# andreicuceu/vega

Measured on AMD Instinct MI355X. Metric: model+chi2 evals/sec (Lya auto+cross), higher is better.
Workload: dtype f64

## Files before the change

vega_amd/csrc/vegamx.hip:

```cpp
#include "vmx_device.h"
#include "vmx_fit.h"
#include "vmx_ensemble.h"
#include "vmx_nested.h"
#include "vmx_smc.h"

#include <atomic>
#include <cmath>
#include <chrono>
#include <thread>
#include <algorithm>
#include <cstdio>
#include <cstdlib>
#include <cstring>
#include <map>
#include <mutex>
#include <queue>
#include <utility>
#include <string>
#include <vector>

#ifndef VMX_MAX_LANES
#define VMX_MAX_LANES 2
#endif

// ... 1566 lines not shown
    DevBuf<double> xtab_key;
    int n_xtab = 0;
    int const_hint = 0;
    int fv_n = 0;
    struct GkSpec { double rp, rt, mock_rp, mock_rt; };
    std::vector<GkSpec> gk_tables;
    std::vector<double> h_k, h_mu;

    int n_coef = 0, ncp = 0, n_knots = 0;
    DevBuf<double> op;
    bool op_set[VMX_MAX_ELL] = {false, false, false, false};
    bool extrapolate = false;
    double x0[VMX_MAX_ELL] = {0}, h[VMX_MAX_ELL] = {0};

    std::vector<PipeDev> pipes;
    std::vector<double> h_r, h_mu_c, h_z, h_relz, h_lnrelz, h_lnrelz2, h_growth;
    DevBuf<double> cr, cmu, crp, crt, cz, crelz, clnrelz, clnrelz2, cgrowth;
    DevBuf<PipeDev> d_pipes;
    std::vector<PkGroup> pk_groups;
    DevBuf<PkGroup> d_pk_groups;
    std::vector<int32_t> pk_members, pk_poly, pk_static;
    DevBuf<int32_t> d_pk_members, d_pk_poly, d_pk_static, d_pipe_active;
    DevBuf<double> poly_coef, poly_bins;
    int64_t poly_bins_total = 0;
    int n_active = 0;
    bool poly_dirty = true;

    std::vector<ItemHost*> items;
    std::vector<MetalHost*> metals;
    DevBuf<ItemDev> d_items;
    DevBuf<MetalDev> d_metals;
    std::vector<double> h_bb, h_odd, h_odd_op;
    std::map<int, int64_t> odd_op_off;
    DevBuf<double> bb_basis, odd_coef, odd_op, odd_dyn, sn_a;
    int sn_n = 0; double sn_tau0 = 0.0, sn_dtau = 1.0;

    std::vector<int32_t> prior_slot;
    std::vector<double> prior_mean, prior_sigma;
    DevBuf<int32_t> d_prior_slot;
    DevBuf<double> d_prior_mean, d_prior_sigma;

    DevBuf<double> gcinv, gres, gz;
    int g_n = 0, g_ld = 0;

    int n_params = 0, max_batch = 0, model_size = 0, slab_rows = 0;
    int pad_l = 0, pad_r = 0;
// ... 574 lines not shown
    for (size_t i = 0; i < e->gk_tables.size(); ++i) {
        const auto& g = e->gk_tables[i];
        if (g.rp == bin_size_rp && g.rt == bin_size_rt && g.mock_rp == mock_size_rp && g.mock_rt == mock_size_rt) return (int)i;
    }
    e->gk_tables.push_back({bin_size_rp, bin_size_rt, mock_size_rp, mock_size_rt});
    return (int)e->gk_tables.size() - 1;
}

int vmx_add_gk_table(vmx_engine* e, double bin_size_rp, double bin_size_rt)
{
    return vmx_add_gk_table_mock(e, bin_size_rp, bin_size_rt, 0.0, 0.0);
}

int vmx_add_pipeline(vmx_engine* e, const vmx_pipe_desc* desc, int32_t n, const double* r, const double* mu,
                     const double* z, const double* rel_z_evol, const double* xi_growth)
{
    if (!e || e->finalized || !desc || n <= 0) return fail(-1, "invalid argument: vmx_add_pipeline");
    if (desc->n_ell < 1 || desc->n_ell > VMX_MAX_ELL) return fail(-1, "invalid argument: n_ell");
    if (desc->gk_table >= (int)e->gk_tables.size()) return fail(-1, "invalid argument: gk_table id");
    if (desc->mock_los_slot >= 0 && !(desc->mock_los_size > 0.0)) return fail(-1, "invalid argument: mock_los_size");
    if (desc->n_smooth < 0 || desc->n_smooth > VMX_MAX_SMOOTH) return fail(-1, "invalid argument: n_smooth");
    PipeDev p{};
    p.d = *desc;
    p.poly_basis = -1; p.col = -1; p.poly_bins_off = -1; p.odd_dyn_off = -1;
    if (!p.d.same_tracer && ((!p.d.tracer[0].is_lya && p.d.tracer[1].is_lya) ||
                             (p.d.tracer[0].is_lya == p.d.tracer[1].is_lya && p.d.tracer[0].discrete &&
                              !p.d.tracer[1].discrete))) {
        std::swap(p.d.tracer[0], p.d.tracer[1]);
        p.tracers_swapped = 1;
    }
    p.n = n;
    p.coord_off = (int64_t)e->h_r.size();
    e->h_r.insert(e->h_r.end(), r, r + n);
    e->h_mu_c.insert(e->h_mu_c.end(), mu, mu + n);
    e->h_z.insert(e->h_z.end(), z, z + n);
    e->h_relz.insert(e->h_relz.end(), rel_z_evol, rel_z_evol + n);
    for (int i = 0; i < n; ++i) { e->h_lnrelz.push_back(std::log(rel_z_evol[i])); e->h_lnrelz2.push_back(std::log(rel_z_evol[i])); }
    p.rp_absmin = 1e300; p.rp_absmax = 0.0; p.rt_min = 1e300; p.rt_max = 0.0;
    for (int i = 0; i < n; ++i) {
        if (r[i] == 0.0) continue;
        const double rp = std::fabs(r[i] * mu[i]), rt = r[i] * std::sqrt(std::max(0.0, 1.0 - mu[i] * mu[i]));
        p.rp_absmin = std::min(p.rp_absmin, rp); p.rp_absmax = std::max(p.rp_absmax, rp);
        p.rt_min = std::min(p.rt_min, rt); p.rt_max = std::max(p.rt_max, rt);
    }
    if (p.rp_absmin > p.rp_absmax) { p.rp_absmin = 0.0; p.rt_min = 0.0; }
    e->h_growth.insert(e->h_growth.end(), xi_growth, xi_growth + n);
    e->pipes.push_back(p);
// ... 407 lines not shown
    REQUIRE(e && invcov && n > 0, "vmx_set_global_invcov");
    drop_lane(e);
    HIP_OK(hipSetDevice(e->device));
    const std::vector<double> half = half_form(invcov, n);
    if (e->finalized) {
        REQUIRE(e->g_n == n, "global inverse covariance size changed");
        HIP_OK(hipStreamSynchronize(e->stream));
        HIP_OK(hipMemcpy2D(e->gcinv.p, (size_t)e->g_ld * sizeof(double), half.data(), (size_t)n * sizeof(double),
                           (size_t)n * sizeof(double), n, hipMemcpyHostToDevice));
        return 0;
    }
    e->g_n = n; e->g_ld = vmx_pad(n);
    return upload_padded(e->gcinv, half.data(), n, n, e->g_ld);
}

int vmx_add_prior(vmx_engine* e, int32_t slot, double mean, double sigma)
{
    REQUIRE(e && !e->finalized && slot >= 0 && sigma != 0.0, "vmx_add_prior");
    e->prior_slot.push_back(slot); e->prior_mean.push_back(mean); e->prior_sigma.push_back(sigma);
    return 0;
}

static int poly_basis_build(vmx_engine* e);
static int xi_sum_plan(vmx_engine* e);

int vmx_finalize(vmx_engine* e, int32_t n_params, int32_t max_batch)
{
    REQUIRE(e && !e->finalized, "vmx_finalize");
    REQUIRE(n_params > 0 && max_batch > 0, "n_params / max_batch");
    REQUIRE(e->nk > 0 && !e->pipes.empty() && !e->items.empty(), "template, pipelines and items are required");
    REQUIRE(e->items.size() <= 16, "at most 16 correlation items");
    REQUIRE(e->pipes.size() * sizeof(PipeDev) <= 48 * 1024, "too many pipelines for the prologue's descriptor stage");
    for (int i = 0; i < VMX_MAX_ELL; ++i) REQUIRE(e->op_set[i], "all four FFTLog operators are required");
    HIP_OK(hipSetDevice(e->device));
    const int Bm = max_batch;
    e->n_params = n_params; e->max_batch = Bm;
    e->slab_rows = Bm > 1024 ? Bm : 1024;
    e->fact_slab_rows = std::max(1024, std::min(4 * Bm, 8192));
    if (getenv("VMX_NO_GRAPH")) e->use_graphs = false;
    if (getenv("VMX_TRACE_HOST")) e->trace_host = true;
    {
        int cus = 256;
        if (hipDeviceGetAttribute(&cus, hipDeviceAttributeMultiprocessorCount, e->device) != hipSuccess || cus <= 0) { (void)hipGetLastError(); cus = 256; }
        e->quad_blocks = 2 * cus;
    }
    if (getenv("VMX_NO_TAB2")) e->no_tab2 = true;
// ... 390 lines not shown
    if (getenv("VMX_NO_DONE_WORD") || hipHostGetDevicePointer((void**)&e->dpin_done, e->pin_done, 0) != hipSuccess) { (void)hipGetLastError(); e->dpin_done = nullptr; }
    if (!getenv("VMX_NO_ZERO_COPY") &&
        (hipHostGetDevicePointer((void**)&e->dpin_theta, e->pin_theta, 0) != hipSuccess ||
         hipHostGetDevicePointer((void**)&e->dpin_chi2, e->pin_chi2, 0) != hipSuccess ||
         hipHostGetDevicePointer((void**)&e->dpin_status, e->pin_status, 0) != hipSuccess)) {
        (void)hipGetLastError();
        e->dpin_theta = nullptr; e->dpin_chi2 = nullptr; e->dpin_status = nullptr;
    }

    e->quad_eligible = e->gcinv.p == nullptr && e->items.size() <= 16;
    for (auto* it : e->items) {
        int na = 0;
        if (it->dev.n_bb[VMX_BB_POST_MUL]) e->quad_eligible = false;
        for (int q = 0; q < it->dev.n_bb[VMX_BB_POST_ADD]; ++q) {
            if (it->dev.bb[VMX_BB_POST_ADD][q].func != VMX_BB_POLY) e->quad_eligible = false;
            na += it->dev.bb[VMX_BB_POST_ADD][q].n_coef;
        }
        if (na > VMX_MAX_QUAD_COEF) e->quad_eligible = false;
    }
    if (getenv("VMX_NO_QUAD")) e->quad_eligible = false;

    HIP_OK(hipStreamSynchronize(e->stream));
    e->finalized = true;
    if (poly_basis_build(e) || xi_sum_plan(e)) { e->finalized = false; return -2; }
    return 0;
}

int vmx_model_size(vmx_engine* e) { return e ? e->model_size : -1; }

int vmx_pipeline_column(vmx_engine* e, int32_t pipeline)
{
    REQUIRE(e && e->finalized && pipeline >= 0 && pipeline < (int)e->pipes.size(), "vmx_pipeline_column");
    return e->pipes[pipeline].col >= 0 ? e->pipes[pipeline].col : -3 - e->n_active;
}

constexpr double QUAD_ENTRY_STAGES = 4.0, QUAD_SKEW = 0.12;
constexpr bool QUAD_K_BANDS = true;

static vmx_engine::QuadList* quad_build_tape(vmx_engine* e, int B)
{
    const int tn = (B + GEMM_BN - 1) / GEMM_BN;
    std::vector<vmx_plan::TapeProblem> probs;
    for (auto* it : e->items) probs.push_back({it->dev.nq, it->dev.nq_pad});
    vmx_plan::Tape T = vmx_plan::plan_quad_tape(probs, tn, e->quad_blocks, QUAD_ENTRY_STAGES, QUAD_SKEW, GEMM_BM, GEMM_BK, QUAD_K_BANDS);
    auto* ql = new vmx_engine::QuadList();
    ql->n_blocks = T.n_blocks;
    ql->n_entries = (int)T.n_slots;
// ... 111 lines not shown
        DevBuf<int32_t> d_ok;
        if (d_ok.upload(ok.data(), ok.size())) return -2;
        int max_n = 0;
        for (int p : e->pk_static) max_n = std::max(max_n, (int)e->pipes[p].n);
        hipLaunchKernelGGL(k_poly_bins, dim3((max_n + 255) / 256, ns, 3), dim3(256), 0, e->stream, e->dev, e->d_pk_static.p,
                           e->poly_bins.p, d_ok.p);
        e->route_setup |= VMX_ROUTE_POLY_BINS;
        HIP_OK(hipGetLastError());
        HIP_OK(hipStreamSynchronize(e->stream));
        HIP_OK(hipMemcpy(ok.data(), d_ok.p, ok.size() * sizeof(int32_t), hipMemcpyDeviceToHost));
        bool changed = false;
        for (int sb = 0; sb < ns; ++sb)
            if (!ok[sb] && e->pipes[e->pk_static[sb]].poly_bins_off >= 0) { e->pipes[e->pk_static[sb]].poly_bins_off = -1; changed = true; }
        if (changed) HIP_OK(hipMemcpy(e->d_pipes.p, e->pipes.data(), e->pipes.size() * sizeof(PipeDev), hipMemcpyHostToDevice));
    }
    HIP_OK(hipStreamSynchronize(e->stream));
    for (int p : e->pk_static) (e->pipes[p].poly_bins_off >= 0 ? e->xi_static_bins : e->xi_static_taps).push_back(p);
    std::vector<int32_t> a = e->xi_static_taps, b = e->xi_static_bins;
    a.push_back(-1); b.push_back(-1);
    if (e->d_xi_static_taps.upload(a.data(), a.size()) || e->d_xi_static_bins.upload(b.data(), b.size())) return -2;
    return 0;
}

static void launch_metal_kron(vmx_engine* e, const EngineDev& D, ItemHost* it, int B)
{
    int item = 0;
    for (size_t q = 0; q < e->items.size(); ++q) if (e->items[q] == it) item = (int)q;
    size_t shmem = 0;
    for (auto* m : it->metals) {
        if (!m->dev.kron_a) continue;
        const int n = m->dev.kron_nrp * m->dev.kron_nrt;
        shmem = std::max(shmem, (size_t)(2 * n + std::max(m->dev.kron_nrp * m->dev.kron_nrp, m->dev.kron_nrt * m->dev.kron_nrt)) * sizeof(double));
    }
    if (shmem == 0) return;
    ScopedTimer t(e, KC_METAL);
    if (!e->kron_attr) { (void)hipFuncSetAttribute((const void*)k_metal_kron, hipFuncAttributeMaxDynamicSharedMemorySize, 160 * 1024); e->kron_attr = true; }
    hipLaunchKernelGGL(k_metal_kron, dim3(B, (unsigned)it->metals.size()), dim3(256), shmem, e->cur, D, item, B);
}

static bool xi_plain_args(vmx_engine* e, XiPlainArgs& A)
{
    if (e->items.size() > VMX_MAX_GROUP || e->extrapolate || e->direct) return false;
    for (size_t q = 0; q < e->items.size(); ++q) {
        const ItemHost* it = e->items[q];
        const ItemDev& d = it->dev;
        if (!it->lean_pair || d.add_vec || d.n_bb[VMX_BB_PRE_MUL] || d.n_bb[VMX_BB_PRE_ADD]) return false;
        const PipeDev& Ps = e->pipes[d.d.pipe_smooth];
        const PipeDev& Pp = e->pipes[d.d.pipe_peak];
        if (Ps.d.n_ell != Pp.d.n_ell || Ps.d.single_ell >= 0 || Pp.d.single_ell >= 0 || Ps.col < 0 || Pp.col < 0) return false;
        XiPlainItem& I = A.it[q];
        I.coord_off = Pp.coord_off; I.q_x0 = it->q_x0.p; I.q_x = it->q_x.p;
        I.n_model = d.d.n_model; I.nq = d.nq; I.nq_pad = d.nq_pad; I.pipe_s = d.d.pipe_smooth; I.pipe_p = d.d.pipe_peak;
        I.col_s = Ps.col; I.col_p = Pp.col; I.n_ell = Ps.d.n_ell; I.split_evol = Pp.split_evol; I.bao_slot = d.d.bao_amp_slot;
        I.item = (int32_t)q;
        I.radiation = Ps.d.radiation;
    }
    return true;
}

static int xi_sum_plan(vmx_engine* e)
{
    e->sums_dirty = false;
    e->lean_groups.clear(); e->static_groups.clear(); e->static_single.clear(); e->lean_single.clear();
    e->sums_any = false;
    const int np = (int)e->pipes.size();
    struct Role { int item = -1, fkind = 0, findex = 0, metal = -1, refs = 0; bool plain = true; };
    std::vector<Role> role(np);
    int metal_base = 0;
    for (int q = 0; q < (int)e->items.size(); ++q) {
        const ItemHost* it = e->items[q];
        const vmx_item_desc& d = it->dev.d;
        auto take = [&](int p, int fkind, int findex, int metal, bool plain) {
            if (p < 0 || p >= np) return;
            Role& r = role[p];
            r.refs += 1; r.item = q; r.fkind = fkind; r.findex = findex; r.metal = metal; r.plain = r.plain && plain;
        };
        take(d.pipe_smooth, 0, 0, -1, true);
        if (d.pipe_peak != d.pipe_smooth) take(d.pipe_peak, 1, d.bao_amp_slot, -1, true);
// ... 3101 lines not shown
    }
    else if (what == 6) { src = e->scal.p; count = (int64_t)B * (int64_t)e->pipes.size() * VMX_NS; }
    else if (what == 7) {
        static_assert(VMX_DEBUG_NS == VMX_NS, "vegamx.h states the row length of the scalars");
#define VMX_SCALAR_INDEX(name) S_##name,
        const int idx[] = {VMX_NS, VMX_DEBUG_SCALARS(VMX_SCALAR_INDEX)};
#undef VMX_SCALAR_INDEX
        const int64_t n = sizeof(idx) / sizeof(idx[0]);
        if (capacity < n) { fail(-1, "invalid argument: capacity too small"); return -1; }
        for (int64_t i = 0; i < n; ++i) out[i] = idx[i];
        return n;
    }
    else if (what == 8) {
        if (index < 0 || index >= (int)e->pipes.size()) { fail(-1, "invalid argument: pipeline index"); return -1; }
        const PipeDev& P = e->pipes[index];
        const double* arr[8] = {e->cr.p, e->crp.p, e->crt.p, e->cz.p, e->crelz.p, e->clnrelz.p, e->clnrelz2.p, e->cgrowth.p};
        if ((int64_t)8 * P.n > capacity) { fail(-1, "invalid argument: capacity too small"); return -1; }
        for (int a = 0; a < 8; ++a)
            if (hipMemcpy(out + (size_t)a * P.n, arr[a] + P.coord_off, (size_t)P.n * sizeof(double), hipMemcpyDeviceToHost) != hipSuccess) { fail(-2, "hipMemcpy"); return -2; }
        return (int64_t)8 * P.n;
    }
    else if (what == 9) {
        if (index < 0 || index >= (int)e->pipes.size()) { fail(-1, "invalid argument: pipeline index"); return -1; }
        if (capacity < 30) { fail(-1, "invalid argument: capacity too small"); return -1; }
        const EngineDev& D = e->dev;
        const PipeDev& P = e->pipes[index];
        int64_t n = 0;
        out[n++] = D.n_coef; out[n++] = D.ncp; out[n++] = D.same_grid; out[n++] = D.extrapolate; out[n++] = e->n_active;
        for (int l = 0; l < VMX_MAX_ELL; ++l) { out[n++] = D.x0[l]; out[n++] = D.h[l]; out[n++] = D.inv_h[l]; out[n++] = D.xlast[l]; }
        out[n++] = P.col; out[n++] = P.n; out[n++] = P.n_pad; out[n++] = P.split_evol; out[n++] = P.poly_basis;
        out[n++] = P.poly_bins_off >= 0 ? 1 : 0; out[n++] = P.odd_x0; out[n++] = P.odd_h; out[n++] = P.odd_ncoef;
        return n;
    }
    else if (what == 10 || what == 11) {
        if (index < 0 || index >= (int)e->items.size()) { fail(-1, "invalid argument: item index"); return -1; }
        const ItemHost* it = e->items[index];
        if (e->last_full || e->last_form == 0 || !it->q_x.p || !it->q_x0.p) { fail(-1, "the last evaluation was not a chi2-only evaluation of the quadratic form: no x' - x0'"); return -1; }
        src = what == 10 ? it->q_x.p : it->q_x0.p; count = (what == 10 ? (int64_t)B : 1) * it->dev.nq_pad;
    }
    else if (what == 12) {
        if (index < 0 || index >= (int)e->pipes.size()) { fail(-1, "invalid argument: pipeline index"); return -1; }
        const PipeDev& P = e->pipes[index];
        if (P.poly_bins_off < 0 || !e->poly_bins.p) { fail(-1, "none: the pipeline has no static basis on its bins"); return -1; }
        src = e->poly_bins.p + P.poly_bins_off; count = (int64_t)3 * P.n_pad;
    }
    else if (what == 13 || what == 14 || what == 18 || what == 19) {
        const bool lean = what < 18, describe = what == 13 || what == 18;
        const int ng = (int)(lean ? e->lean_groups.size() : e->static_groups.size());
        if (describe && (index < 0 || index >= ng)) {
            if (capacity < 1) { fail(-1, "invalid argument: capacity too small"); return -1; }
            out[0] = ng;
            return 1;
        }
        if (index < 0 || index >= ng) { fail(-1, "invalid argument: group index"); return -1; }
// ... 141 lines not shown
```

vega_amd/csrc/vmx_device.h:

```cpp
#pragma once
#include <hip/hip_runtime.h>
#include <stdint.h>
#include "../../include/vegamx.h"
#include "vmx_plan.h"

#define VMX_NS 40
#define VMX_PAD 32
#define VMX_MAX_BB 32
#define VMX_MAX_METALS 64
#define VMX_MAX_QUAD_COEF 64
#define VMX_MAX_GROUP 8
#define VMX_MAX_MARG 16

enum {
    S_BIAS1 = 0, S_BB1, S_BIAS2, S_BB2,
    S_UV_BG, S_UV_BP, S_UV_LAM, S_HE_BG, S_HE_LAM,
    S_HCD_B, S_HCD_BB, S_HCD_L0,
    S_GA, S_GB, S_EA, S_EB,
    S_AQ1, S_AQ2, S_AKV, S_AAV, S_ABV, S_AKP,
    S_VD1, S_VD2,
    S_AP, S_AT, S_DRP, S_EV1A, S_EV1B, S_EV2A, S_EV2B,
    S_RAD_S, S_RAD_A, S_RAD_L, S_RAD_D, S_RAD_IL, S_RAD_ID,
    S_NO_RULE
};

static inline int vmx_pad(int n) { return (n + VMX_PAD - 1) / VMX_PAD * VMX_PAD; }

struct PipeDev {
    vmx_pipe_desc d;
    int32_t n;
    int32_t n_pad;
    int64_t coord_off;
    int64_t xi_off;
    double rp_absmin, rp_absmax, rt_min, rt_max;
    int32_t col;
    int32_t poly_basis;
    int64_t poly_bins_off;
    int32_t split_evol;
    int32_t tracers_swapped;
    int32_t odd_rel, odd_asy, odd_ncoef;
    int32_t odd_slot[5];
    int64_t odd_off;
    int64_t odd_dyn_off;
    int32_t odd_dyn_ld;
    double odd_x0, odd_h;
};

struct BBTermDev {
    int32_t func, n_coef;
    int32_t slot[16];
    int64_t basis_off;
};

struct MetalDev {
    vmx_metal_desc d;
    int64_t mat_off;
    int32_t mat_ld;
    int64_t xim_off;
    const double* svec;
    const double* basis;
// ... 56 lines not shown
    const double* mu;
    const double* mu_img;
    vmx_plan::MuTierDesc mu_tier[vmx_plan::MU_TIERS];
    const double* mu_img_w;
    const double* sq1mmu2;
    const double* lnmu;
    const double* wl;
    const double* fv_x; const double* fv_f; int32_t fv_n;
    const double* gk;
    double* xtab;
    const int32_t* const_slots; int32_t n_const_slots;
    const int32_t* xtab_pipe; const int32_t* xtab_partner; int32_t n_xtab; int32_t xtab_level; double* xtab_key; double* xtab_k;
    int32_t xtab_block0;
    const double* gk_mom;
    int32_t n_gk;
    int32_t n_coef, ncp;
    int32_t extrapolate;
    double x0[VMX_MAX_ELL], h[VMX_MAX_ELL], xlast[VMX_MAX_ELL], inv_h[VMX_MAX_ELL];
    int same_grid;
    int32_t n_pipe;
    int32_t n_active;
    const double* poly_coef;
    const double* poly_bins;
    int32_t n_static;
    const PipeDev* pipes;
    const double* crp; const double* crt;
    const double* cr; const double* cmu; const double* cz; const double* crelz; const double* clnrelz; const double* cgrowth;
    const double* clnrelz2;
    int32_t n_items;
    const ItemDev* items;
    const MetalDev* metals;
    int32_t n_metals_total;
    const double* bb_basis;
    const double* odd_coef;
    const double* odd_dyn;
    const double* sn_a; int32_t sn_n; double sn_tau0, sn_dtau;
    int32_t n_priors;
    const int32_t* prior_slot; const double* prior_mean; const double* prior_sigma;
    int32_t n_params;
    const double* theta;
    const double* theta_host; double* theta_copy; double* chi2_host; int32_t* status_host;
    int32_t src_host;
    double* scal;
    double* metal_bias;
    double beta_override; int32_t beta_override_on;
    double* pl;
// ... 2702 lines not shown
                const double v = (part[tid][0] + part[tid][1]) + (part[tid][2] + part[tid][3]);
                pr = sx[r] * (2.0 * (v - g.lin[r]));
            }
            for (int off = 32; off > 0; off >>= 1) pr += __shfl_down(pr, off, 64);
            if (tid == 0) {
                *(volatile double*)&g.part[blockIdx.x] = pr;
                if (blockIdx.x == 0 && item) {
                    *(volatile int32_t*)D.status_host = D.status[0];
                    D.k_live[2] = D.coef_win[0]; D.k_live[3] = D.coef_win[1]; D.coef_win[0] = 0x7fffffff; D.coef_win[1] = -1;
                    xtab_key_store(D);
                }
            }
        }
        return;
    }
    if (tid < t) {
        const int r = blockIdx.x + tid * gridDim.x;
        const double v = (part[tid][0] + part[tid][1]) + (part[tid][2] + part[tid][3]);
        if constexpr (FUSED) post_bin(D, D.items[item], 0, r, v);
        else Dp[r] = v;
    }
}

__device__ inline double legendre_even(int e, double x)
{
    const double x2 = x * x;
    switch (e) {
        case 0: return 1.0;
        case 1: return 0.5 * (3.0 * x2 - 1.0);
        case 2: return 0.125 * ((35.0 * x2 - 30.0) * x2 + 3.0);
        default: return 0.0625 * (((231.0 * x2 - 315.0) * x2 + 105.0) * x2 - 5.0);
    }
}

template <bool STATIC_BASIS>
__device__ __forceinline__ double spline_legendre(const EngineDev& D, const PipeDev& P, int b, int nB, double x, double rmu,
                                                  double a0, double a1, double a2, bool& oob)
{
    const vmx_pipe_desc& d = P.d;
    const int n_ell = d.n_ell, single_ell = d.single_ell;
    const size_t ncols = (size_t)nB * D.n_active;
    const size_t col = (size_t)(P.col >= 0 ? P.col : 0) * nB + b;
    const double* cf[4];
    double tt[4];
    bool on[4];
#pragma unroll
    for (int e = 0; e < 4; ++e) {
        const int ee = e < n_ell ? e : 0;
        const bool inside = D.extrapolate || !(x < D.x0[ee] || x > D.xlast[ee]);
        on[e] = e < n_ell && inside;
        if (e < n_ell && !inside) oob = true;
        const double u = (x - D.x0[ee]) * D.inv_h[ee];
        int j = (int)floor(u);
        if (j < 0) j = 0;
        if (j > D.n_coef - 4) j = D.n_coef - 4;
        if (!(u == u)) j = 0;
        tt[e] = u - (double)j;
        cf[e] = STATIC_BASIS ? D.poly_coef + ((size_t)ee * D.n_static + P.poly_basis) * 3 * D.ncp + j
                             : D.coef + ((size_t)ee * ncols + col) * D.ncp + j;
    }
    double tap[4][4];
    if (STATIC_BASIS) {
#pragma unroll
        for (int e = 0; e < 4; ++e)
#pragma unroll
            for (int q = 0; q < 4; ++q)
                tap[e][q] = fma(a2, cf[e][2 * D.ncp + q], fma(a1, cf[e][D.ncp + q], a0 * cf[e][q]));
    } else {
#pragma unroll
        for (int e = 0; e < 4; ++e)
#pragma unroll
            for (int q = 0; q < 4; ++q) tap[e][q] = cf[e][q];
    }
    double xi = 0.0;
#pragma unroll
    for (int e = 0; e < 4; ++e) {
        const double t = tt[e], t2 = t * t, t3 = t2 * t;
        const double omt = 1.0 - t;
        const double w0 = omt * omt * omt;
        const double w1 = 3.0 * t3 - 6.0 * t2 + 4.0;
        const double w2 = -3.0 * t3 + 3.0 * t2 + 3.0 * t + 1.0;
        const double s = (tap[e][0] * w0 + tap[e][1] * w1 + tap[e][2] * w2 + tap[e][3] * t3) * (1.0 / 6.0);
        if (on[e]) {
            if (single_ell >= 0) { if (e == single_ell) xi = s; }
            else xi += s * legendre_even(e, rmu);
        }
    }
    return xi;
}

__device__ __forceinline__ void kaiser_coefficients(const vmx_pipe_desc& d, const double* sc, double& a0, double& a1, double& a2)
{
    double c01 = sc[S_BIAS1], c02 = sc[S_BIAS2];
    const double c11 = sc[S_BB1], c12 = d.same_tracer ? sc[S_BB1] : sc[S_BB2];
    if (d.same_tracer) c02 = c01;
    a0 = c01 * c02; a1 = fma(c01, c12, c11 * c02); a2 = c11 * c12;
}

template <int MODE>
__device__ __forceinline__ double xi_bin_value(const EngineDev& D, int p, int b, int bin, int nB, bool& oob_out)
{
    const PipeDev& P = D.pipes[p];
    const vmx_pipe_desc& d = P.d;
    const double* sc = D.scal + ((size_t)b * D.n_pipe + p) * VMX_NS;
    const size_t c = P.coord_off + bin;
    const double r = D.cr[c], rp0 = D.crp[c], rt0 = D.crt[c];
    const double lnrelz = D.clnrelz[c], growth = D.cgrowth[c];
    const double drp = sc[S_DRP], s_ap = sc[S_AP], s_at = sc[S_AT];
// ... 106 lines not shown
    bool oob;
    D.xi[P.xi_off + (size_t)b * P.n_pad + bin] = xi_bin_value<2>(D, p, b, bin, (int)gridDim.z, oob);
}

__global__ __launch_bounds__(256) void k_poly_bins(EngineDev D, const int32_t* pipes, double* out, int32_t* ok)
{
    const int sb = blockIdx.y, p = pipes[sb], i = blockIdx.z;
    const PipeDev& P = D.pipes[p];
    const int bin = blockIdx.x * 256 + threadIdx.x;
    if (bin >= P.n || P.poly_bins_off < 0) return;
    const size_t c = P.coord_off + bin;
    const double r = D.cr[c], rp0 = D.crp[c], rt0 = D.crt[c];
    double xi = 0.0;
    bool oob = false;
    if (r != 0.0) {
        const double rr2 = fma(rp0, rp0, rt0 * rt0);
        if (rr2 != 0.0)
            xi = spline_legendre<true>(D, P, 0, 1, 0.5 * log(rr2), rp0 * vmx_rsqrt(rr2), i == 0 ? 1.0 : 0.0, i == 1 ? 1.0 : 0.0,
                                       i == 2 ? 1.0 : 0.0, oob);
    }
    if (oob) ok[sb] = 0;
    out[P.poly_bins_off + (size_t)i * P.n_pad + bin] = xi;
}

__global__ __launch_bounds__(256) void k_xi_assemble_quad(EngineDev D, int item0, int store_xi)
{
    const ItemDev& it = D.items[item0 + blockIdx.z];
    const int b = blockIdx.y, nB = gridDim.y;
    const int i = blockIdx.x * 256 + threadIdx.x;
    if (i >= it.nq_pad) return;
    const double* t = D.theta + (size_t)b * D.n_params;
    double v = 0.0;
    if (i < it.d.n_model) {
        const PipeDev& Pp = D.pipes[it.d.pipe_peak];
        const PipeDev& Ps = D.pipes[it.d.pipe_smooth];
        bool oob_p, oob_s;
        double xs, xp;
        if (it.plain_pair) {
            const size_t c = Pp.coord_off + i;
            const double r = D.cr[c], rp0 = D.crp[c], rt0 = D.crt[c];
            const double* scp = D.scal + ((size_t)b * D.n_pipe + it.d.pipe_peak) * VMX_NS;
            const double* scs = D.scal + ((size_t)b * D.n_pipe + it.d.pipe_smooth) * VMX_NS;
            const double ev = (Pp.split_evol ? vmx_exp(fma(scp[S_EV1A], D.clnrelz[c], scp[S_EV2A] * D.clnrelz2[c]))
                                             : vmx_exp((scp[S_EV1A] + scp[S_EV2A]) * D.clnrelz[c])) * D.cgrowth[c];
            xs = 0.0; xp = 0.0; oob_p = false; oob_s = false;
            if (r != 0.0) {
#pragma unroll
                for (int half = 0; half < 2; ++half) {
                    const double* sc = half ? scp : scs;
                    const double rrp = sc[S_AP] * (rp0 + sc[S_DRP]), rrt = sc[S_AT] * rt0;
                    const double rr2 = fma(rrp, rrp, rrt * rrt);
                    if (rr2 != 0.0) {
                        const double v = spline_legendre<false>(D, half ? Pp : Ps, b, nB, 0.5 * vmx_log(rr2), rrp * vmx_rsqrt(rr2),
                                                                0.0, 0.0, 0.0, half ? oob_p : oob_s);
                        if (half) xp = v * ev; else xs = v * ev;
                    }
                }
            }
        } else {
            xs = xi_bin_value<0>(D, it.d.pipe_smooth, b, i, nB, oob_s);
            xp = xi_bin_value<0>(D, it.d.pipe_peak, b, i, nB, oob_p);
        }
        if (oob_p || oob_s) atomicOr(&D.status[b], VMX_STATUS_BOUNDS);
        if (store_xi) {
            D.xi[Ps.xi_off + (size_t)b * Ps.n_pad + i] = xs;
            D.xi[Pp.xi_off + (size_t)b * Pp.n_pad + i] = xp;
        }
        const double bao = t[it.d.bao_amp_slot];
        v = fma(bao, xp, xs);
        if (it.add_vec) v = fma(it.add_slot >= 0 ? t[it.add_slot] : it.add_default, it.add_vec[i], v);
        if (it.n_bb[VMX_BB_PRE_MUL]) v *= bb_total(D, it, VMX_BB_PRE_MUL, t, i, it.d.n_model);
        if (it.n_bb[VMX_BB_PRE_ADD]) v += (1.0 + bao) * bb_total(D, it, VMX_BB_PRE_ADD, t, i, it.d.n_model);
        v -= it.q_x0[i];
    } else if (i < it.nq) {
        v = (1.0 + t[it.d.bao_amp_slot]) * t[it.q_slot[i - it.d.n_model]] - it.q_x0[i];
    }
    it.q_x[(size_t)b * it.nq_pad + i] = v;
}

struct XiPlainItem { int64_t coord_off; const double* q_x0; double* q_x; int32_t n_model, nq, nq_pad, pipe_s, pipe_p, col_s, col_p,
                     n_ell, split_evol, bao_slot, item, radiation; };
struct XiPlainArgs { XiPlainItem it[VMX_MAX_GROUP]; };

template <bool SAME>
__device__ __forceinline__ double xi_plain_spline(const EngineDev& D, const double* coef_col, size_t ell_stride, int n_ell, double x,
                                                  double rmu, bool& oob)
{
    const double* cf[4];
    double tt[4];
    bool on[4];
    if (SAME) {
        const bool inside = !(x < D.x0[0] || x > D.xlast[0]);
        if (!inside) oob = true;
        const double u = (x - D.x0[0]) * D.inv_h[0];
        int j = (int)floor(u);
        if (j < 0) j = 0;
        if (j > D.n_coef - 4) j = D.n_coef - 4;
        if (!(u == u)) j = 0;
        const double t = u - (double)j;
#pragma unroll
        for (int e = 0; e < 4; ++e) {
            on[e] = e < n_ell && inside;
            tt[e] = t;
            cf[e] = coef_col + (size_t)(e < n_ell ? e : 0) * ell_stride + j;
        }
    } else {
#pragma unroll
        for (int e = 0; e < 4; ++e) {
            const int ee = e < n_ell ? e : 0;
            const bool inside = !(x < D.x0[ee] || x > D.xlast[ee]);
            on[e] = e < n_ell && inside;
            if (e < n_ell && !inside) oob = true;
            const double u = (x - D.x0[ee]) * D.inv_h[ee];
            int j = (int)floor(u);
            if (j < 0) j = 0;
            if (j > D.n_coef - 4) j = D.n_coef - 4;
            if (!(u == u)) j = 0;
            tt[e] = u - (double)j;
            cf[e] = coef_col + (size_t)ee * ell_stride + j;
        }
    }
    double tap[4][4];
#pragma unroll
    for (int e = 0; e < 4; ++e)
#pragma unroll
        for (int q = 0; q < 4; ++q) tap[e][q] = cf[e][q];
    double xi = 0.0;
    const double x2 = rmu * rmu;
#pragma unroll
    for (int e = 0; e < 4; ++e) {
        const double t = tt[e], t2 = t * t, t3 = t2 * t;
        const double omt = 1.0 - t;
        const double w0 = omt * omt * omt;
        const double w1 = 3.0 * t3 - 6.0 * t2 + 4.0;
        const double w2 = -3.0 * t3 + 3.0 * t2 + 3.0 * t + 1.0;
        const double sp = (tap[e][0] * w0 + tap[e][1] * w1 + tap[e][2] * w2 + tap[e][3] * t3) * (1.0 / 6.0);
        const double leg = e == 0 ? 1.0 : e == 1 ? 0.5 * (3.0 * x2 - 1.0) : e == 2 ? 0.125 * ((35.0 * x2 - 30.0) * x2 + 3.0)
                                        : 0.0625 * (((231.0 * x2 - 315.0) * x2 + 105.0) * x2 - 5.0);
        if (on[e]) xi += sp * leg;
    }
    return xi;
}

template <int NW, bool SAME>
__global__ __launch_bounds__(256) void k_xi_quad_plain(EngineDev D, XiPlainArgs A, int item0, int B)
{
    const XiPlainItem& I = A.it[item0 + blockIdx.z];
    const int i = blockIdx.x * 256 + threadIdx.x;
    if (i >= I.nq_pad) return;
    const int b0 = blockIdx.y * NW;
    if (i >= I.n_model) {
        const ItemDev& it = D.items[I.item];
#pragma unroll
        for (int w = 0; w < NW; ++w) {
            const int b = b0 + w;
            if (b >= B) break;
            const double* t = D.theta + (size_t)b * D.n_params;
            double v = 0.0;
            if (i < I.nq) v = (1.0 + t[I.bao_slot]) * t[it.q_slot[i - I.n_model]] - I.q_x0[i];
            I.q_x[(size_t)b * I.nq_pad + i] = v;
        }
        return;
    }
    const size_t c = (size_t)I.coord_off + i;
    const double r = D.cr[c], rp0 = D.crp[c], rt0 = D.crt[c], lnz = D.clnrelz[c], growth = D.cgrowth[c], x0v = I.q_x0[i];
    const double lnz2 = I.split_evol ? D.clnrelz2[c] : 0.0;
    const size_t ncols = (size_t)B * D.n_active, ell_stride = ncols * D.ncp;
    double out[NW];
    bool oob[NW];
#pragma unroll
    for (int w = 0; w < NW; ++w) {
        const int b = min(b0 + w, B - 1);
        const double* scs = D.scal + ((size_t)b * D.n_pipe + I.pipe_s) * VMX_NS;
        const double* scp = D.scal + ((size_t)b * D.n_pipe + I.pipe_p) * VMX_NS;
        const double ev = (I.split_evol ? vmx_exp(fma(scp[S_EV1A], lnz, scp[S_EV2A] * lnz2)) : vmx_exp((scp[S_EV1A] + scp[S_EV2A]) * lnz)) * growth;
        double xs = 0.0, xp = 0.0;
        oob[w] = false;
        if (r != 0.0) {
#pragma unroll
            for (int half = 0; half < 2; ++half) {
                const double* sc = half ? scp : scs;
                const double rrp = sc[S_AP] * (rp0 + sc[S_DRP]), rrt = sc[S_AT] * rt0;
                const double rr2 = fma(rrp, rrp, rrt * rrt);
                if (rr2 != 0.0) {
                    const double* col = D.coef + ((size_t)(half ? I.col_p : I.col_s) * B + b) * D.ncp;
                    const double v = xi_plain_spline<SAME>(D, col, ell_stride, I.n_ell, 0.5 * vmx_log(rr2), rrp * vmx_rsqrt(rr2), oob[w]);
                    if (half) xp = v * ev; else xs = v * ev;
                }
            }
        }
        if (I.radiation) {
            const bool resc = I.radiation == 2;
            const double drp = scs[S_DRP];
            const double rp = resc ? fma(scs[S_AP], rp0 + drp, drp) : rp0 + drp;
            const double rtr = resc ? scs[S_AT] * rt0 : rt0;
            const double rs2 = fma(rp, rp, rtr * rtr);
            const double irs = vmx_rsqrt(rs2);
            const double rs = rs2 * irs, ms = rp * irs;
            double xr = scs[S_RAD_S] * (irs * irs) * (1.0 - scs[S_RAD_A] * (1.0 - ms * ms));
            xr *= vmx_exp(-rs * fma(1.0 + ms, scs[S_RAD_IL], scs[S_RAD_ID]));
            xs += xr;
        }
        const double bao = D.theta[(size_t)b * D.n_params + I.bao_slot];
        out[w] = fma(bao, xp, xs) - x0v;
    }
#pragma unroll
    for (int w = 0; w < NW; ++w) {
        const int b = b0 + w;
        if (b >= B) break;
        if (oob[w]) atomicOr(&D.status[b], VMX_STATUS_BOUNDS);
        I.q_x[(size_t)b * I.nq_pad + i] = out[w];
    }
}
// ... 250 lines not shown
```

vega_amd/engine.py:

```python
import ctypes as C
import os
from pathlib import Path

import numpy as np

from . import fftlog_op, static_terms

_LIB_PATH = Path(__file__).resolve().parent / 'libvegamx.so'
_lib = None

VMX_MAX_ELL = 4
VMX_MAX_SMOOTH = 3
VMX_N_KERNELS = 13
HCD = {'none': 0, 'Rogers': 1, 'sinc': 2, 'fvoigt': 3}
NL = {'none': 0, 'arinyo': 1, 'mcdonald': 2}
VD = {None: 0, 'gauss': 1, 'lorentz': 2}
SCALE_UNIT, SCALE_AP_AT, SCALE_AISO_EPS, SCALE_PHI_ALPHA = 0, 1, 2, 3
PKLIN = {'peak': 0, 'smooth': 1, 'full': 2}
MAT_DISTORTION, MAT_INVCOV, MAT_METAL = 0, 1, 2
BB_POS = {('pre', 'mul'): 0, ('pre', 'add'): 1, ('post', 'mul'): 2, ('post', 'add'): 3}
BB_POLY, BB_SKY = 0, 1
DEFAULT_GROWTH_RATE = 0.970386

STATUS_BOUNDS, STATUS_ARINYO, STATUS_NONFINITE, STATUS_NOT_CONSTANT = 1, 2, 4, 8
# ... 1507 lines not shown
        return {name for name, bit in self.ROUTE_BITS.items() if mask & bit}

    def bins_scalar_index(self):
        idx = self.debug_read(7, 0, 32).astype(int)
        names = ('NS',) + self.BINS_SCALAR_NAMES
        assert idx.size == len(names)
        return dict(zip(names, idx.tolist()))

    def bins_scalars(self, B):
        ns = self.bins_scalar_index()['NS']
        return self.debug_read(6, 0, B * self.n_pipelines * ns).reshape(B, self.n_pipelines, ns).copy()

    def bins_static(self, pid):
        n = int(self.bins_grid(pid)['n'])
        arr = self.debug_read(8, pid, 8 * n).reshape(8, n)
        return {name: arr[i].copy() for i, name in enumerate(self.BINS_STATIC_NAMES)}

    def bins_grid(self, pid):
        g = self.debug_read(9, pid, 32)
        out = dict(n_coef=int(g[0]), ncp=int(g[1]), same_grid=bool(g[2]), extrapolate=bool(g[3]), n_columns=int(g[4]))
        per_ell = g[5:21].reshape(4, 4)
        out.update(x0=per_ell[:, 0].copy(), h=per_ell[:, 1].copy(), inv_h=per_ell[:, 2].copy(), xlast=per_ell[:, 3].copy())
        out.update(column=int(g[21]), n=int(g[22]), n_pad=int(g[23]), split_evol=bool(g[24]), static_basis=int(g[25]),
                   static_bins=bool(g[26]), odd_x0=float(g[27]), odd_h=float(g[28]), odd_ncoef=int(g[29]))
        return out

    def bins_coefficients(self, B):
        g = self.bins_grid(0)
        return self.debug_read(2, 0, 4 * B * g['n_columns'] * g['ncp']).reshape(4, g['n_columns'], B, g['ncp']).copy()

    def bins_xi(self, pid, B):
        g = self.bins_grid(pid)
        return self.debug_read(1, pid, B * g['n_pad']).reshape(B, g['n_pad']).copy()

    def quad_vector(self, name, B):
        qi = self.item_names.index(name)
        x0 = self.debug_read(11, qi, self.prob.items[name].model_grid.size + 128).copy()
        return self.debug_read(10, qi, B * x0.size).reshape(B, x0.size).copy(), x0

    def lean_groups(self, static=False):
        what = 18 if static else 13
        n_groups = int(self.debug_read(what, -1, 1)[0])
        out = []
        for g in range(n_groups):
            d = self.debug_read(what, g, 64)
            members = [tuple(int(v) for v in d[5 + 3 * m:8 + 3 * m]) for m in range(int(d[1]))]
            out.append(dict(n=int(d[2]), n_pad=int(d[3]), presum=bool(d[4]), members=members))
# ... 111 lines not shown
```

Measured before the change: 966,200.

## Precompute static spline knot indices, weights and Legendre factors for unscaled pipelines

For pipelines with unit scale mode, no drp shift and no odd/relativistic terms, the spline coordinates do not depend on the parameters. A finalize-time kernel now tabulates, per bin and multipole, the knot index, the cubic B-spline weights and the Legendre factor. The xi assembly kernels then read these tables instead of recomputing log, rsqrt, floor and polynomials on every evaluation. The spline and Legendre code is also factored into helpers with explicit fma and contraction turned off, presumably to keep results bitwise identical. The cost is extra table memory traffic (20 doubles plus 5 ints per bin), traded against the transcendental and polynomial arithmetic it replaces.

```diff
diff --git a/vega_amd/csrc/vegamx.hip b/vega_amd/csrc/vegamx.hip
--- a/vega_amd/csrc/vegamx.hip
+++ b/vega_amd/csrc/vegamx.hip
@@ -1612,6 +1612,7 @@
     std::vector<int32_t> pk_members, pk_poly, pk_static;
     DevBuf<int32_t> d_pk_members, d_pk_poly, d_pk_static, d_pipe_active;
     DevBuf<double> poly_coef, poly_bins;
+    DevBuf<double> xi_tab; DevBuf<int32_t> xi_tab_j;
     int64_t poly_bins_total = 0;
     int n_active = 0;
     bool poly_dirty = true;
@@ -2232,7 +2233,7 @@
     if (desc->n_smooth < 0 || desc->n_smooth > VMX_MAX_SMOOTH) return fail(-1, "invalid argument: n_smooth");
     PipeDev p{};
     p.d = *desc;
-    p.poly_basis = -1; p.col = -1; p.poly_bins_off = -1; p.odd_dyn_off = -1;
+    p.poly_basis = -1; p.col = -1; p.poly_bins_off = -1; p.xi_tab_off = -1; p.odd_dyn_off = -1;
     if (!p.d.same_tracer && ((!p.d.tracer[0].is_lya && p.d.tracer[1].is_lya) ||
                              (p.d.tracer[0].is_lya == p.d.tracer[1].is_lya && p.d.tracer[0].discrete &&
                               !p.d.tracer[1].discrete))) {
@@ -2686,6 +2687,7 @@
 }
 
 static int poly_basis_build(vmx_engine* e);
+static int xi_static_build(vmx_engine* e);
 static int xi_sum_plan(vmx_engine* e);
 
 int vmx_finalize(vmx_engine* e, int32_t n_params, int32_t max_batch)
@@ -3122,7 +3124,7 @@
 
     HIP_OK(hipStreamSynchronize(e->stream));
     e->finalized = true;
-    if (poly_basis_build(e) || xi_sum_plan(e)) { e->finalized = false; return -2; }
+    if (poly_basis_build(e) || xi_static_build(e) || xi_sum_plan(e)) { e->finalized = false; return -2; }
     return 0;
 }
 
@@ -3280,6 +3282,41 @@
     return 0;
 }
 
+static int xi_static_build(vmx_engine* e)
+{
+    std::vector<int32_t> cand;
+    int64_t total = 0;
+    int max_n = 0;
+    for (int p = 0; p < (int)e->pipes.size(); ++p) {
+        PipeDev& pd = e->pipes[p];
+        const vmx_pipe_desc& d = pd.d;
+        pd.xi_tab_off = -1;
+        if (getenv("VMX_NO_XI_STATIC") || pd.col < 0 || d.scale_mode != VMX_SCALE_UNIT || d.drp_slot >= 0 || pd.odd_rel || pd.odd_asy ||
+            d.radiation == 2 || d.single_ell >= 0 || pd.n <= 0) continue;
+        pd.xi_tab_off = total;
+        total += vmx_pad(pd.n);
+        max_n = std::max(max_n, (int)pd.n);
+        cand.push_back(p);
+    }
+    if (cand.empty()) return 0;
+    std::vector<int32_t> ok(cand.size(), 1);
+    DevBuf<int32_t> d_cand, d_ok;
+    if (e->xi_tab.alloc((size_t)20 * total, true) || e->xi_tab_j.alloc((size_t)5 * total, true) ||
+        d_cand.upload(cand.data(), cand.size()) || d_ok.upload(ok.data(), ok.size())) return -2;
+    e->dev.xi_tab = e->xi_tab.p; e->dev.xi_tab_j = e->xi_tab_j.p;
+    HIP_OK(hipMemcpy(e->d_pipes.p, e->pipes.data(), e->pipes.size() * sizeof(PipeDev), hipMemcpyHostToDevice));
+    hipLaunchKernelGGL(k_xi_static_tab, dim3((max_n + 255) / 256, (unsigned)cand.size()), dim3(256), 0, e->stream, e->dev, d_cand.p,
+                       e->xi_tab.p, e->xi_tab_j.p, d_ok.p);
+    HIP_OK(hipGetLastError());
+    HIP_OK(hipStreamSynchronize(e->stream));
+    HIP_OK(hipMemcpy(ok.data(), d_ok.p, ok.size() * sizeof(int32_t), hipMemcpyDeviceToHost));
+    bool changed = false;
+    for (size_t q = 0; q < cand.size(); ++q)
+        if (!ok[q]) { e->pipes[cand[q]].xi_tab_off = -1; changed = true; }
+    if (changed) HIP_OK(hipMemcpy(e->d_pipes.p, e->pipes.data(), e->pipes.size() * sizeof(PipeDev), hipMemcpyHostToDevice));
+    return 0;
+}
+
 static void launch_metal_kron(vmx_engine* e, const EngineDev& D, ItemHost* it, int B)
 {
     int item = 0;
@@ -3312,6 +3349,9 @@
         I.col_s = Ps.col; I.col_p = Pp.col; I.n_ell = Ps.d.n_ell; I.split_evol = Pp.split_evol; I.bao_slot = d.d.bao_amp_slot;
         I.item = (int32_t)q;
         I.radiation = Ps.d.radiation;
+        I.tab_s = Ps.xi_tab_off; I.tab_p = Pp.xi_tab_off; I.tab_ld = Ps.n_pad;
+        if (Pp.n_pad != Ps.n_pad || I.n_model > Pp.n) I.tab_p = -1;
+        if (I.n_model > Ps.n) I.tab_s = -1;
     }
     return true;
 }
@@ -6459,7 +6499,7 @@
     }
     else if (what == 9) {
         if (index < 0 || index >= (int)e->pipes.size()) { fail(-1, "invalid argument: pipeline index"); return -1; }
-        if (capacity < 30) { fail(-1, "invalid argument: capacity too small"); return -1; }
+        if (capacity < 31) { fail(-1, "invalid argument: capacity too small"); return -1; }
         const EngineDev& D = e->dev;
         const PipeDev& P = e->pipes[index];
         int64_t n = 0;
@@ -6467,6 +6507,7 @@
         for (int l = 0; l < VMX_MAX_ELL; ++l) { out[n++] = D.x0[l]; out[n++] = D.h[l]; out[n++] = D.inv_h[l]; out[n++] = D.xlast[l]; }
         out[n++] = P.col; out[n++] = P.n; out[n++] = P.n_pad; out[n++] = P.split_evol; out[n++] = P.poly_basis;
         out[n++] = P.poly_bins_off >= 0 ? 1 : 0; out[n++] = P.odd_x0; out[n++] = P.odd_h; out[n++] = P.odd_ncoef;
+        out[n++] = P.xi_tab_off >= 0 ? 1 : 0;
         return n;
     }
     else if (what == 10 || what == 11) {
diff --git a/vega_amd/csrc/vmx_device.h b/vega_amd/csrc/vmx_device.h
--- a/vega_amd/csrc/vmx_device.h
+++ b/vega_amd/csrc/vmx_device.h
@@ -36,6 +36,7 @@
     int32_t col;
     int32_t poly_basis;
     int64_t poly_bins_off;
+    int64_t xi_tab_off;
     int32_t split_evol;
     int32_t tracers_swapped;
     int32_t odd_rel, odd_asy, odd_ncoef;
@@ -138,6 +139,7 @@
     int32_t n_active;
     const double* poly_coef;
     const double* poly_bins;
+    const double* xi_tab; const int32_t* xi_tab_j;
     int32_t n_static;
     const PipeDev* pipes;
     const double* crp; const double* crt;
@@ -2886,15 +2888,44 @@
     }
 }
 
-__device__ inline double legendre_even(int e, double x)
-{
+__device__ __forceinline__ double legendre_even(int e, double x)
+{
+#pragma clang fp contract(off)
     const double x2 = x * x;
     switch (e) {
         case 0: return 1.0;
-        case 1: return 0.5 * (3.0 * x2 - 1.0);
-        case 2: return 0.125 * ((35.0 * x2 - 30.0) * x2 + 3.0);
-        default: return 0.0625 * (((231.0 * x2 - 315.0) * x2 + 105.0) * x2 - 5.0);
-    }
+        case 1: return 0.5 * fma(3.0, x2, -1.0);
+        case 2: return 0.125 * fma(fma(35.0, x2, -30.0), x2, 3.0);
+        default: return 0.0625 * fma(fma(fma(231.0, x2, -315.0), x2, 105.0), x2, -5.0);
+    }
+}
+
+struct SplineKnot { int j; double w0, w1, w2, t3; bool inside; };
+
+__device__ __forceinline__ SplineKnot spline_knot(const EngineDev& D, int ee, double x)
+{
+#pragma clang fp contract(off)
+    SplineKnot K;
+    K.inside = !(x < D.x0[ee] || x > D.xlast[ee]);
+    const double u = (x - D.x0[ee]) * D.inv_h[ee];
+    int j = (int)floor(u);
+    if (j < 0) j = 0;
+    if (j > D.n_coef - 4) j = D.n_coef - 4;
+    if (!(u == u)) j = 0;
+    K.j = j;
+    const double t = u - (double)j, t2 = t * t, t3 = t2 * t;
+    const double omt = 1.0 - t;
+    K.w0 = omt * omt * omt;
+    K.w1 = fma(3.0, t3, fma(-6.0, t2, 4.0));
+    K.w2 = fma(-3.0, t3, fma(3.0, t2, fma(3.0, t, 1.0)));
+    K.t3 = t3;
+    return K;
+}
+
+__device__ __forceinline__ double spline_tap_sum(double c0, double c1, double c2, double c3, double w0, double w1, double w2, double t3)
+{
+#pragma clang fp contract(off)
+    return fma(c3, t3, fma(c2, w2, fma(c1, w1, c0 * w0))) * (1.0 / 6.0);
 }
 
 template <bool STATIC_BASIS>
@@ -2906,20 +2937,16 @@
     const size_t ncols = (size_t)nB * D.n_active;
     const size_t col = (size_t)(P.col >= 0 ? P.col : 0) * nB + b;
     const double* cf[4];
-    double tt[4];
+    SplineKnot K[4];
     bool on[4];
 #pragma unroll
     for (int e = 0; e < 4; ++e) {
         const int ee = e < n_ell ? e : 0;
-        const bool inside = D.extrapolate || !(x < D.x0[ee] || x > D.xlast[ee]);
+        K[e] = spline_knot(D, ee, x);
+        const bool inside = D.extrapolate || K[e].inside;
         on[e] = e < n_ell && inside;
         if (e < n_ell && !inside) oob = true;
-        const double u = (x - D.x0[ee]) * D.inv_h[ee];
-        int j = (int)floor(u);
-        if (j < 0) j = 0;
-        if (j > D.n_coef - 4) j = D.n_coef - 4;
-        if (!(u == u)) j = 0;
-        tt[e] = u - (double)j;
+        const int j = K[e].j;
         cf[e] = STATIC_BASIS ? D.poly_coef + ((size_t)ee * D.n_static + P.poly_basis) * 3 * D.ncp + j
                              : D.coef + ((size_t)ee * ncols + col) * D.ncp + j;
     }
@@ -2939,15 +2966,10 @@
     double xi = 0.0;
 #pragma unroll
     for (int e = 0; e < 4; ++e) {
-        const double t = tt[e], t2 = t * t, t3 = t2 * t;
-        const double omt = 1.0 - t;
-        const double w0 = omt * omt * omt;
-        const double w1 = 3.0 * t3 - 6.0 * t2 + 4.0;
-        const double w2 = -3.0 * t3 + 3.0 * t2 + 3.0 * t + 1.0;
-        const double s = (tap[e][0] * w0 + tap[e][1] * w1 + tap[e][2] * w2 + tap[e][3] * t3) * (1.0 / 6.0);
+        const double s = spline_tap_sum(tap[e][0], tap[e][1], tap[e][2], tap[e][3], K[e].w0, K[e].w1, K[e].w2, K[e].t3);
         if (on[e]) {
             if (single_ell >= 0) { if (e == single_ell) xi = s; }
-            else xi += s * legendre_even(e, rmu);
+            else xi = fma(s, legendre_even(e, rmu), xi);
         }
     }
     return xi;
@@ -3100,6 +3122,9 @@
     if (oob) ok[sb] = 0;
     out[P.poly_bins_off + (size_t)i * P.n_pad + bin] = xi;
 }
+
+__device__ __forceinline__ double xi_static_value(const EngineDev& D, int64_t off, int ld, int bin, const double* coef_col,
+                                                  size_t ell_stride, int n_ell);
 
 __global__ __launch_bounds__(256) void k_xi_assemble_quad(EngineDev D, int item0, int store_xi)
 {
@@ -3125,11 +3150,18 @@
             if (r != 0.0) {
 #pragma unroll
                 for (int half = 0; half < 2; ++half) {
+                    const PipeDev& P = half ? Pp : Ps;
+                    if (P.xi_tab_off >= 0 && i < P.n) {
+                        const double v = xi_static_value(D, P.xi_tab_off, P.n_pad, i, D.coef + ((size_t)P.col * nB + b) * D.ncp,
+                                                         (size_t)nB * D.n_active * D.ncp, P.d.n_ell);
+                        if (half) xp = v * ev; else xs = v * ev;
+                        continue;
+                    }
                     const double* sc = half ? scp : scs;
                     const double rrp = sc[S_AP] * (rp0 + sc[S_DRP]), rrt = sc[S_AT] * rt0;
                     const double rr2 = fma(rrp, rrp, rrt * rrt);
                     if (rr2 != 0.0) {
-                        const double v = spline_legendre<false>(D, half ? Pp : Ps, b, nB, 0.5 * vmx_log(rr2), rrp * vmx_rsqrt(rr2),
+                        const double v = spline_legendre<false>(D, P, b, nB, 0.5 * vmx_log(rr2), rrp * vmx_rsqrt(rr2),
                                                                 0.0, 0.0, 0.0, half ? oob_p : oob_s);
                         if (half) xp = v * ev; else xs = v * ev;
                     }
@@ -3157,7 +3189,8 @@
 }
 
 struct XiPlainItem { int64_t coord_off; const double* q_x0; double* q_x; int32_t n_model, nq, nq_pad, pipe_s, pipe_p, col_s, col_p,
-                     n_ell, split_evol, bao_slot, item, radiation; };
+                     n_ell, split_evol, bao_slot, item, radiation, tab_ld;
+                     int64_t tab_s, tab_p; };
 struct XiPlainArgs { XiPlainItem it[VMX_MAX_GROUP]; };
 
 template <bool SAME>
@@ -3165,37 +3198,25 @@
                                                   double rmu, bool& oob)
 {
     const double* cf[4];
-    double tt[4];
+    SplineKnot K[4];
     bool on[4];
     if (SAME) {
-        const bool inside = !(x < D.x0[0] || x > D.xlast[0]);
-        if (!inside) oob = true;
-        const double u = (x - D.x0[0]) * D.inv_h[0];
-        int j = (int)floor(u);
-        if (j < 0) j = 0;
-        if (j > D.n_coef - 4) j = D.n_coef - 4;
-        if (!(u == u)) j = 0;
-        const double t = u - (double)j;
+        const SplineKnot K0 = spline_knot(D, 0, x);
+        if (!K0.inside) oob = true;
 #pragma unroll
         for (int e = 0; e < 4; ++e) {
-            on[e] = e < n_ell && inside;
-            tt[e] = t;
-            cf[e] = coef_col + (size_t)(e < n_ell ? e : 0) * ell_stride + j;
+            on[e] = e < n_ell && K0.inside;
+            K[e] = K0;
+            cf[e] = coef_col + (size_t)(e < n_ell ? e : 0) * ell_stride + K0.j;
         }
     } else {
 #pragma unroll
         for (int e = 0; e < 4; ++e) {
             const int ee = e < n_ell ? e : 0;
-            const bool inside = !(x < D.x0[ee] || x > D.xlast[ee]);
-            on[e] = e < n_ell && inside;
-            if (e < n_ell && !inside) oob = true;
-            const double u = (x - D.x0[ee]) * D.inv_h[ee];
-            int j = (int)floor(u);
-            if (j < 0) j = 0;
-            if (j > D.n_coef - 4) j = D.n_coef - 4;
-            if (!(u == u)) j = 0;
-            tt[e] = u - (double)j;
-            cf[e] = coef_col + (size_t)ee * ell_stride + j;
+            K[e] = spline_knot(D, ee, x);
+            on[e] = e < n_ell && K[e].inside;
+            if (e < n_ell && !K[e].inside) oob = true;
+            cf[e] = coef_col + (size_t)ee * ell_stride + K[e].j;
         }
     }
     double tap[4][4];
@@ -3204,20 +3225,87 @@
 #pragma unroll
         for (int q = 0; q < 4; ++q) tap[e][q] = cf[e][q];
     double xi = 0.0;
-    const double x2 = rmu * rmu;
 #pragma unroll
     for (int e = 0; e < 4; ++e) {
-        const double t = tt[e], t2 = t * t, t3 = t2 * t;
-        const double omt = 1.0 - t;
-        const double w0 = omt * omt * omt;
-        const double w1 = 3.0 * t3 - 6.0 * t2 + 4.0;
-        const double w2 = -3.0 * t3 + 3.0 * t2 + 3.0 * t + 1.0;
-        const double sp = (tap[e][0] * w0 + tap[e][1] * w1 + tap[e][2] * w2 + tap[e][3] * t3) * (1.0 / 6.0);
-        const double leg = e == 0 ? 1.0 : e == 1 ? 0.5 * (3.0 * x2 - 1.0) : e == 2 ? 0.125 * ((35.0 * x2 - 30.0) * x2 + 3.0)
-                                        : 0.0625 * (((231.0 * x2 - 315.0) * x2 + 105.0) * x2 - 5.0);
-        if (on[e]) xi += sp * leg;
+        const double sp = spline_tap_sum(tap[e][0], tap[e][1], tap[e][2], tap[e][3], K[e].w0, K[e].w1, K[e].w2, K[e].t3);
+        if (on[e]) xi = fma(sp, legendre_even(e, rmu), xi);
     }
     return xi;
+}
+
+template <int NW, int G>
+__device__ __forceinline__ void xi_static_spline(const EngineDev& D, int64_t off, int ld, int bin, const double* const (&col)[NW],
+                                                 size_t ell_stride, int n_ell, double (&xi)[NW], bool& live)
+{
+    const int32_t* tj = D.xi_tab_j + 5 * (size_t)off + bin;
+    const double* tw = D.xi_tab + 20 * (size_t)off + bin;
+    live = tj[(size_t)4 * ld] != 0;
+#pragma unroll
+    for (int w = 0; w < NW; ++w) xi[w] = 0.0;
+#pragma unroll
+    for (int g = 0; g < 4; g += G) {
+        int j[G];
+        double wt[G][5], tap[NW][G][4];
+#pragma unroll
+        for (int q = 0; q < G; ++q) j[q] = tj[(size_t)(g + q) * ld];
+#pragma unroll
+        for (int q = 0; q < G; ++q)
+#pragma unroll
+            for (int f = 0; f < 5; ++f) wt[q][f] = tw[(size_t)(5 * (g + q) + f) * ld];
+#pragma unroll
+        for (int w = 0; w < NW; ++w)
+#pragma unroll
+            for (int q = 0; q < G; ++q)
+#pragma unroll
+                for (int t = 0; t < 4; ++t) tap[w][q][t] = col[w][(size_t)(g + q < n_ell ? g + q : 0) * ell_stride + j[q] + t];
+#pragma unroll
+        for (int q = 0; q < G; ++q)
+#pragma unroll
+            for (int w = 0; w < NW; ++w) {
+                const double sp = spline_tap_sum(tap[w][q][0], tap[w][q][1], tap[w][q][2], tap[w][q][3], wt[q][0], wt[q][1], wt[q][2], wt[q][3]);
+                if (g + q < n_ell && live) xi[w] = fma(sp, wt[q][4], xi[w]);
+            }
+        if (g + G < 4) __builtin_amdgcn_sched_barrier(0);
+    }
+}
+
+__device__ __forceinline__ double xi_static_value(const EngineDev& D, int64_t off, int ld, int bin, const double* coef_col,
+                                                  size_t ell_stride, int n_ell)
+{
+    const double* const col[1] = {coef_col};
+    double xi[1];
+    bool live;
+    xi_static_spline<1, 1>(D, off, ld, bin, col, ell_stride, n_ell, xi, live);
+    return xi[0];
+}
+
+__global__ __launch_bounds__(256) void k_xi_static_tab(EngineDev D, const int32_t* pipes, double* tab, int32_t* tab_j, int32_t* ok)
+{
+    const int sb = blockIdx.y;
+    const PipeDev& P = D.pipes[pipes[sb]];
+    const int bin = blockIdx.x * 256 + threadIdx.x;
+    if (bin >= P.n || P.xi_tab_off < 0) return;
+    const size_t c = P.coord_off + bin, ld = P.n_pad;
+    const double r = D.cr[c], rp0 = D.crp[c], rt0 = D.crt[c];
+    const double rrp = 1.0 * (rp0 + 0.0), rrt = 1.0 * rt0;
+    const double rr2 = fma(rrp, rrp, rrt * rrt);
+    const bool live = r != 0.0 && rr2 != 0.0;
+    int32_t* tj = tab_j + 5 * (size_t)P.xi_tab_off + bin;
+    double* tw = tab + 20 * (size_t)P.xi_tab_off + bin;
+    tj[4 * ld] = live ? 1 : 0;
+    double x = 0.0, rmu = 0.0;
+    if (live) { x = 0.5 * vmx_log(rr2); rmu = rrp * vmx_rsqrt(rr2); }
+    for (int e = 0; e < 4; ++e) {
+        const bool on = live && e < P.d.n_ell;
+        const SplineKnot K = spline_knot(D, e < P.d.n_ell ? e : 0, x);
+        if (on && !K.inside) ok[sb] = 0;
+        tj[e * ld] = on ? K.j : 0;
+        tw[(5 * e + 0) * ld] = on ? K.w0 : 0.0;
+        tw[(5 * e + 1) * ld] = on ? K.w1 : 0.0;
+        tw[(5 * e + 2) * ld] = on ? K.w2 : 0.0;
+        tw[(5 * e + 3) * ld] = on ? K.t3 : 0.0;
+        tw[(5 * e + 4) * ld] = on ? legendre_even(e, rmu) : 0.0;
+    }
 }
 
 template <int NW, bool SAME>
@@ -3244,29 +3332,48 @@
     const double r = D.cr[c], rp0 = D.crp[c], rt0 = D.crt[c], lnz = D.clnrelz[c], growth = D.cgrowth[c], x0v = I.q_x0[i];
     const double lnz2 = I.split_evol ? D.clnrelz2[c] : 0.0;
     const size_t ncols = (size_t)B * D.n_active, ell_stride = ncols * D.ncp;
-    double out[NW];
-    bool oob[NW];
+    double out[NW], xc[2][NW];
+    bool oob[NW], has[2][NW];
+#pragma unroll
+    for (int w = 0; w < NW; ++w) { xc[0][w] = 0.0; xc[1][w] = 0.0; has[0][w] = false; has[1][w] = false; oob[w] = false; }
+    if (r != 0.0) {
+#pragma unroll
+        for (int half = 0; half < 2; ++half) {
+            const int64_t tab = half ? I.tab_p : I.tab_s;
+            const int pipe = half ? I.pipe_p : I.pipe_s, ccol = half ? I.col_p : I.col_s;
+            if (tab >= 0) {
+                const double* col[NW];
+                double v[NW];
+                bool live;
+#pragma unroll
+                for (int w = 0; w < NW; ++w) col[w] = D.coef + ((size_t)ccol * B + min(b0 + w, B - 1)) * D.ncp;
+                xi_static_spline<NW, SAME ? 1 : 2>(D, tab, I.tab_ld, i, col, ell_stride, I.n_ell, v, live);
+#pragma unroll
+                for (int w = 0; w < NW; ++w) { xc[half][w] = v[w]; has[half][w] = live; }
+            } else {
+#pragma unroll
+                for (int w = 0; w < NW; ++w) {
+                    const int b = min(b0 + w, B - 1);
+                    const double* sc = D.scal + ((size_t)b * D.n_pipe + pipe) * VMX_NS;
+                    const double rrp = sc[S_AP] * (rp0 + sc[S_DRP]), rrt = sc[S_AT] * rt0;
+                    const double rr2 = fma(rrp, rrp, rrt * rrt);
+                    if (rr2 != 0.0) {
+                        xc[half][w] = xi_plain_spline<SAME>(D, D.coef + ((size_t)ccol * B + b) * D.ncp, ell_stride, I.n_ell, 0.5 * vmx_log(rr2),
+                                                            rrp * vmx_rsqrt(rr2), oob[w]);
+                        has[half][w] = true;
+                    }
+                }
+            }
+        }
+    }
 #pragma unroll
     for (int w = 0; w < NW; ++w) {
         const int b = min(b0 + w, B - 1);
         const double* scs = D.scal + ((size_t)b * D.n_pipe + I.pipe_s) * VMX_NS;
         const double* scp = D.scal + ((size_t)b * D.n_pipe + I.pipe_p) * VMX_NS;
         const double ev = (I.split_evol ? vmx_exp(fma(scp[S_EV1A], lnz, scp[S_EV2A] * lnz2)) : vmx_exp((scp[S_EV1A] + scp[S_EV2A]) * lnz)) * growth;
-        double xs = 0.0, xp = 0.0;
-        oob[w] = false;
-        if (r != 0.0) {
-#pragma unroll
-            for (int half = 0; half < 2; ++half) {
-                const double* sc = half ? scp : scs;
-                const double rrp = sc[S_AP] * (rp0 + sc[S_DRP]), rrt = sc[S_AT] * rt0;
-                const double rr2 = fma(rrp, rrp, rrt * rrt);
-                if (rr2 != 0.0) {
-                    const double* col = D.coef + ((size_t)(half ? I.col_p : I.col_s) * B + b) * D.ncp;
-                    const double v = xi_plain_spline<SAME>(D, col, ell_stride, I.n_ell, 0.5 * vmx_log(rr2), rrp * vmx_rsqrt(rr2), oob[w]);
-                    if (half) xp = v * ev; else xs = v * ev;
-                }
-            }
-        }
+        double xs = has[0][w] ? xc[0][w] * ev : 0.0;
+        const double xp = has[1][w] ? xc[1][w] * ev : 0.0;
         if (I.radiation) {
             const bool resc = I.radiation == 2;
             const double drp = scs[S_DRP];
diff --git a/vega_amd/engine.py b/vega_amd/engine.py
--- a/vega_amd/engine.py
+++ b/vega_amd/engine.py
@@ -1553,7 +1553,8 @@
         per_ell = g[5:21].reshape(4, 4)
         out.update(x0=per_ell[:, 0].copy(), h=per_ell[:, 1].copy(), inv_h=per_ell[:, 2].copy(), xlast=per_ell[:, 3].copy())
         out.update(column=int(g[21]), n=int(g[22]), n_pad=int(g[23]), split_evol=bool(g[24]), static_basis=int(g[25]),
-                   static_bins=bool(g[26]), odd_x0=float(g[27]), odd_h=float(g[28]), odd_ncoef=int(g[29]))
+                   static_bins=bool(g[26]), odd_x0=float(g[27]), odd_h=float(g[28]), odd_ncoef=int(g[29]),
+                   xi_static=bool(g[30]))
         return out
 
     def bins_coefficients(self, B):
```

New measurement: 968,500 (median of 4 runs). No clear change (+0.2%).
